# matthewhoung/inference-arena

Hardware: AMD Instinct MI355X
Metric: req/sec (whole node) + P50/P99 e2e latency, YOLOv5n→MobileNetV2 at 1/2/4/8 GPU (higher is better)
Workload: dtype fp32

## Files before the change

### csrc/bindings.cpp

```cpp
#include <pybind11/numpy.h>
#include <pybind11/pybind11.h>
#include <pybind11/stl.h>

#include <cstring>
#include <malloc.h>
#include <map>
#include <mutex>

#include "kernels/launch.h"
#include "runtime/executor.h"
#include "runtime/echo_instance.h"
#include "runtime/http_front.h"
#include "runtime/http_loadgen.h"
#include "runtime/ipc_buffer.h"
#include "runtime/peer.h"
#include "runtime/jpeg_decode.h"
#include "runtime/jpeg_ingest.h"
#include "runtime/batcher.h"
#include "runtime/split.h"
#include "runtime/crash_trace.h"

namespace py = pybind11;
using namespace arena;

// ... 28 lines not shown
  p.H = req<int>(d, "H");
  p.W = req<int>(d, "W");
  p.xs = req<int>(d, "xs");
  p.Cin = req<int>(d, "Cin");
  p.w = ptr<const void*>(d, "w");
  p.Kpad = req<int>(d, "Kpad");
  p.bias = ptr<const float*>(d, "bias");
  p.y = ptr<void*>(d, "y");
  p.Ho = req<int>(d, "Ho");
  p.Wo = req<int>(d, "Wo");
  p.ys = req<int>(d, "ys");
  p.Cout = req<int>(d, "Cout");
  p.Cout_pad = req<int>(d, "Cout_pad");
  p.KH = req<int>(d, "KH");
  p.KW = req<int>(d, "KW");
  p.stride = get<int>(d, "stride", 1);
  p.pad_t = get<int>(d, "pad_t", 0);
  p.pad_l = get<int>(d, "pad_l", 0);
  p.res = ptr<const void*>(d, "res");
  p.rs = get<int>(d, "rs", 0);
  p.y2 = ptr<void*>(d, "y2");
  p.y2s = get<int>(d, "y2s", 0);
  p.act = get<int>(d, "act", 0);
  p.f32out = get<int>(d, "f32out", 0);
  p.bdev = ptr<const int*>(d, "bdev");
  p.impl = get<int>(d, "impl", 0);
  p.pw_w = ptr<const void*>(d, "pw_w");
  p.pw_bias = ptr<const float*>(d, "pw_bias");
  p.pw_y = ptr<void*>(d, "pw_y");
  p.pw_ys = get<int>(d, "pw_ys", 0);
  p.pw_cout = get<int>(d, "pw_cout", 0);
  p.pw_kpad = get<int>(d, "pw_kpad", 0);
  p.pw_act = get<int>(d, "pw_act", 0);
  p.w3 = ptr<const void*>(d, "w3");
  p.sk_ws = ptr<float*>(d, "sk_ws");
  p.sk_ws_bytes = get<int64_t>(d, "sk_ws_bytes", 0);
  prepare_kernels();
  if (get<int>(d, "f32", 0))
    conv2d_f32(p, stream_of(d));
  else
    conv2d(p, stream_of(d));
}

void py_dwconv(const py::dict& d) {
  DwParams p{};
  p.x = ptr<const void*>(d, "x");
  p.B = req<int>(d, "B");
  p.H = req<int>(d, "H");
  p.W = req<int>(d, "W");
  p.xs = req<int>(d, "xs");
  p.C = req<int>(d, "C");
  p.w = ptr<const void*>(d, "w");
  p.bias = ptr<const float*>(d, "bias");
  p.y = ptr<void*>(d, "y");
  p.Ho = req<int>(d, "Ho");
  p.Wo = req<int>(d, "Wo");
  p.ys = req<int>(d, "ys");
  p.stride = get<int>(d, "stride", 1);
  p.act = get<int>(d, "act", 0);
  p.bdev = ptr<const int*>(d, "bdev");
  if (get<int>(d, "f32", 0))
    dwconv3x3_f32(p, stream_of(d));
  else
    dwconv3x3(p, stream_of(d));
}

// ... 444 lines not shown
  m.def("crash_trace_installed", &arena::crash_trace_installed);
  m.def("dump_thread_stack", &arena::dump_thread_stack, py::arg("tid"));
  m.def("malloc_trim", []() {
    py::gil_scoped_release nogil;
    return malloc_trim(0) != 0;
  });
  m.def("malloc_info", []() {
    const struct mallinfo2 mi = mallinfo2();
    py::dict d;
    d["arena"] = (uint64_t)mi.arena;
    d["mmapped"] = (uint64_t)mi.hblkhd;
    d["in_use"] = (uint64_t)mi.uordblks;
    d["free"] = (uint64_t)mi.fordblks;
    d["releasable"] = (uint64_t)mi.keepcost;
    return d;
  });
  bind_jpeg(m);
  m.def("conv2d", &py_conv2d);
  m.def("set_conv_impl", &set_conv_impl);
  m.def("get_conv_impl", &get_conv_impl);
  m.def("dwconv3x3", &py_dwconv);
  m.def("sppf_pool", &py_sppf);
  m.def("ir_block", &py_ir_block);
  m.def("c3_block", &py_c3_block);
  m.def("set_conv_pw", &set_conv_pw);
  m.def("set_conv_v3", &set_conv_v3);
  m.def("set_ir_wave", &set_ir_wave);
  m.def("set_irx_parts", &set_irx_parts);
  m.def("set_irx_slices_big", &set_irx_slices_big);
  m.def("set_ir_t14", &set_ir_t14);
  m.def("set_ir_crop", &set_ir_crop);
  m.def("set_ir_s2k16", &set_ir_s2k16);
  m.def("set_ir_crop_split", &set_ir_crop_split);
  m.def("letterbox_s2d", &py_letterbox);
  m.def("detect_decode", &py_decode);
  m.def("yolo_raw", &py_yolo_raw);
  m.def("tensor_in_s2d", &py_tensor_in);
  m.def("nms", &py_nms);
  m.def("crop_plan", &py_crop_plan);
  m.def("crop_gather_s2d", &py_crop_gather);
  m.def("global_avgpool", &py_avgpool);
  m.def("head_pool", &py_head_pool);
  m.def("topk_softmax", &py_topk);
  m.attr("SIZEOF_IMAGE_META") = (int)sizeof(ImageMeta);
  m.attr("SIZEOF_CTRL") = (int)sizeof(Ctrl);
  m.attr("SIZEOF_CANDIDATE") = (int)sizeof(Candidate);
  m.attr("SIZEOF_DETECTION") = (int)sizeof(Detection);
  m.attr("SIZEOF_CROPREF") = (int)sizeof(CropRef);
  m.attr("SIZEOF_TOPK") = (int)sizeof(TopkResult);
  m.attr("OP_FIELDS") = kOpFields;

  py::class_<Executor, std::shared_ptr<Executor>>(m, "Executor")
      .def(py::init([](const py::dict& cfg) { return std::make_shared<Executor>(config_from(cfg)); }))
      .def("set_weights",
           [](Executor& e, py::array_t<uint8_t, py::array::c_style> blob) { e.set_weights(blob.data(), blob.size()); })
      .def("set_weights_device",
           [](Executor& e, uintptr_t ptr, size_t bytes) {
             py::gil_scoped_release nogil;
             e.set_weights_device((const void*)ptr, bytes);
           })
      .def("weights_host",
           [](Executor& e) {
             std::vector<uint8_t> v;
             {
               py::gil_scoped_release nogil;
               v = e.weights_host();
// ... 112 lines not shown
           })
      .def("submit_device",
           [](Executor& e, const std::vector<std::tuple<uintptr_t, int, int, int>>& images,
              const std::vector<py::array_t<float, py::array::c_style | py::array::forcecast>>& boxes) {
             if (images.size() != boxes.size()) throw std::runtime_error("submit_device: one box array per image");
             std::vector<Executor::DeviceImage> imgs;
             std::vector<std::vector<Detection>> dets(images.size());
             for (size_t i = 0; i < images.size(); ++i) {
               Executor::DeviceImage d;
               d.ptr = std::get<0>(images[i]);
               d.h = std::get<1>(images[i]);
               d.w = std::get<2>(images[i]);
               d.device = std::get<3>(images[i]);
               imgs.push_back(d);
               const auto& b = boxes[i];
               if (b.size() == 0) continue;
               if (b.ndim() != 2 || b.shape(1) != 6) throw std::runtime_error("submit_device: boxes must be [k, 6]");
               const float* q = b.data();
               for (ssize_t k = 0; k < b.shape(0); ++k, q += 6) {
                 Detection dd{};
                 dd.x1 = q[0];
                 dd.y1 = q[1];
                 dd.x2 = q[2];
                 dd.y2 = q[3];
                 dd.conf = q[4];
                 dd.cls = (int)q[5];
                 dets[i].push_back(dd);
               }
             }
             py::gil_scoped_release nogil;
             return e.submit_device(imgs, dets);
           })
      .def("conv_choices", &Executor::conv_choices)
      .def("stream", &Executor::stream);

  py::class_<SplitInstance, std::shared_ptr<SplitInstance>>(m, "SplitInstance")
      .def(py::init([](std::shared_ptr<Executor> det, std::shared_ptr<Executor> cls) {
        return std::make_shared<SplitInstance>(det, cls);
      }))
      .def("submit",
           [](SplitInstance& s, const py::list& imgs) {
             std::vector<py::array> keep;
             auto v = images_from(imgs, keep);
             py::gil_scoped_release nogil;
             return s.submit(v);
           })
      .def("collect",
           [](SplitInstance& s, int slot) {
             BatchResult r;
             {
               py::gil_scoped_release nogil;
               r = s.collect(slot);
             }
             return result_to_py(r, s.max_det());
           })
      .def("num_slots", &SplitInstance::num_slots)
      .def("buckets", &SplitInstance::buckets);

  py::class_<JpegSet, std::shared_ptr<JpegSet>>(m, "JpegSet")
      .def(py::init(&make_jpeg_set), py::arg("uploads"), py::arg("pinned") = true,
           "JPEG uploads entropy-decoded once into (pinned) host buffers, for Executor.submit_jpeg_set")
      .def("__len__", [](const JpegSet& s) { return s.items.size(); })
      .def("coef_bytes", [](const JpegSet& s, int i) { return (int64_t)jpeg_payload_bytes(s.items.at(i)->info); })
      .def_property_readonly("pinned", [](const JpegSet& s) {
        for (const auto& it : s.items)
          if (!it->pinned) return false;
// ... 443 lines not shown
```

### csrc/kernels/halo_x3g.hip

```cpp
#include <stdexcept>
#include <string>

#include "common.h"
#include "launch.h"

namespace arena {

namespace {

typedef float f32x16 __attribute__((ext_vector_type(16)));
typedef unsigned u32x4 __attribute__((ext_vector_type(4)));

constexpr int HG_P = 56;

__host__ __device__ constexpr int hg_th(int TW, int WM, int TM) { return WM * TM * (32 / TW); }
__host__ __device__ constexpr int hg_lds_bytes(int TW, int WM, int WN, int TM, int TN) {
  return ((hg_th(TW, WM, TM) + 2) * (TW + 2) + 2 * WN * TN * 32) * HG_P * 2;
}
__host__ __device__ constexpr int hr_lds_bytes(int TW, int WM, int TM) {
  return (hg_th(TW, WM, TM) + 2) * (TW + 2) * HG_P * 2;
}

__device__ __forceinline__ int hg_xcd_remap(int bx, int nx) {
  const int q = nx / 8, r = nx % 8, x = bx % 8, y = bx / 8;
  return (x < r ? x * (q + 1) : r * (q + 1) + (x - r) * q) + y;
}

__device__ __forceinline__ f32x16 hg_mfma_x3(const bf16x8& ah, const bf16x8& am, const bf16x8& al,
                                             const bf16x8& bh, const bf16x8& bm, const bf16x8& bl, f32x16 c) {
  c = __builtin_amdgcn_mfma_f32_32x32x16_bf16(am, bm, c, 0, 0, 0);
  c = __builtin_amdgcn_mfma_f32_32x32x16_bf16(al, bh, c, 0, 0, 0);
  c = __builtin_amdgcn_mfma_f32_32x32x16_bf16(ah, bl, c, 0, 0, 0);
  c = __builtin_amdgcn_mfma_f32_32x32x16_bf16(am, bh, c, 0, 0, 0);
  c = __builtin_amdgcn_mfma_f32_32x32x16_bf16(ah, bm, c, 0, 0, 0);
  return __builtin_amdgcn_mfma_f32_32x32x16_bf16(ah, bh, c, 0, 0, 0);
}

}

template <int TW, int WM, int WN, int TM, int TN, int PWN>
__device__ __forceinline__ void hg_epilogue(const ConvParams& p, f32x16 (&acc)[TM][TN], int b, int oy0, int ox0,
                                            int n0, int wm, int wn, int lane) {
  constexpr int RF = 32 / TW, BN = WN * TN * 32;
  const int fr = lane & 31, fk = 8 * (lane >> 5);
  const int kh4 = 4 * (lane >> 5);
  if constexpr (PWN > 0) {
// ... 96 lines not shown
  }
}

template <int TW, int WM, int WN, int TM, int TN, int PWN = 0>
__global__ __launch_bounds__(WM * WN * 64) void conv_x3hg_kernel(const ConvParams p) {
  static_assert(PWN == 0 || WN == 1, "the fused 1x1 needs every 3x3 channel of a pixel in one wave");
  constexpr int NT = WM * WN * 64;
  constexpr int RF = 32 / TW;
  constexpr int TH = WM * TM * RF;
  constexpr int HC = TW + 2, HPIX = (TH + 2) * HC;
  constexpr int BN = WN * TN * 32;
  constexpr int XI = (HPIX * 4 + NT - 1) / NT;
  constexpr int WI = (BN * 6 + NT - 1) / NT;
  extern __shared__ __attribute__((aligned(16))) bf16 hg_lds[];
  bf16* sX = hg_lds;
  bf16* sW = hg_lds + HPIX * HG_P;

  const int tid = threadIdx.x, lane = tid & 63, wave = tid >> 6;
  const int wm = wave % WM, wn = wave / WM;
  const int tiles_x = (p.Wo + TW - 1) / TW, tiles_y = (p.Ho + TH - 1) / TH;
  const int ntn = (p.Cout_pad + BN - 1) / BN;
  const int per_img = tiles_x * tiles_y * ntn;
  const int bx = hg_xcd_remap(blockIdx.x, gridDim.x);
  const int b = bx / per_img;
  if (b >= live_batch(p.B, p.bdev)) return;
  int t = bx - b * per_img;
  const int nt = t % ntn;
  t /= ntn;
  const int ty = t / tiles_x, tx = t - ty * tiles_x;
  const int oy0 = ty * TH, ox0 = tx * TW, n0 = nt * BN;
  const int iy0 = oy0 - p.pad_t, ix0 = ox0 - p.pad_l;
  const int H = p.H, W = p.W, Cin = p.Cin;

  const __amdgpu_buffer_rsrc_t xr = __builtin_amdgcn_make_buffer_rsrc(
      const_cast<void*>(p.x), (short)0, (int)((size_t)p.B * H * W * p.xs * 4), 0x00020000);
  const int cin32 = (Cin + 31) >> 5;
  const __amdgpu_buffer_rsrc_t wr = __builtin_amdgcn_make_buffer_rsrc(
      const_cast<void*>(p.w3), (short)0, (int)((size_t)9 * cin32 * p.Cout_pad * 192), 0x00020000);
  constexpr int kOob = 0x7fffffff & ~15;

  int x_off[XI];
  const size_t img = (size_t)b * H * W;
#pragma unroll
  for (int j = 0; j < XI; ++j) {
    const int i = tid + NT * j;
    const int px = i >> 2, q = i & 3;
    const int hy = px / HC, hx = px - hy * HC;
    const int iy = iy0 + hy, ix = ix0 + hx;
    const bool in = i < HPIX * 4 && (unsigned)iy < (unsigned)H && (unsigned)ix < (unsigned)W;
    x_off[j] = in ? (int)(((img + (size_t)iy * W + ix) * p.xs + 4 * q) * 4) : kOob;
  }
  int w_off[WI];
#pragma unroll
  for (int j = 0; j < WI; ++j) {
    const int i = tid + NT * j;
    const int row = i / 6, piece = i - (i / 6) * 6;
    const int n = n0 + row;
    w_off[j] = (i < BN * 6 && n < p.Cout_pad) ? (n * 96 + (piece >> 1) * 32 + 8 * (piece & 1)) * 2 : kOob;
  }

  f32x4 rx[XI];
  u32x4 rw[WI];
  auto load_x = [&](int cc) {
#pragma unroll
    for (int j = 0; j < XI; ++j) {
      const int i = tid + NT * j;
// ... 311 lines not shown
  X(1, 16, 4, 1, 1, 2)   \
  X(2, 16, 4, 1, 2, 3)   \
  X(3, 16, 4, 1, 1, 3)   \
  X(4, 16, 4, 1, 1, 5)   \
  X(5, 16, 8, 1, 1, 5)   \
  X(6, 8, 4, 1, 1, 2)    \
  X(7, 8, 4, 1, 1, 5)    \
  X(8, 16, 2, 2, 2, 1)   \
  X(9, 8, 4, 1, 1, 3)

#define HR_PW_VARIANTS(X) \
  X(0, 16, 4, 1, 2, 2)  \
  X(1, 16, 4, 2, 2, 2)  \
  X(2, 16, 4, 1, 3, 3)  \
  X(3, 16, 4, 2, 3, 3)  \
  X(4, 8, 4, 1, 2, 2)   \
  X(5, 8, 4, 1, 3, 3)

}

bool x3hg_supported(const ConvParams& p) {
  const size_t x_bytes = (size_t)p.B * p.H * p.W * p.xs * 4;
  const size_t w_bytes = (size_t)9 * ((p.Cin + 31) / 32) * p.Cout_pad * 192;
  return p.w3 != nullptr && p.KH == 3 && p.KW == 3 && p.stride == 1 && p.Cin % 4 == 0 && p.xs % 4 == 0 &&
         x_bytes < (1u << 31) - (1u << 20) && w_bytes < (1u << 31) - (1u << 20) && p.Cout % 4 == 0 &&
         p.ys % 4 == 0 && (p.res == nullptr || p.rs % 4 == 0) && (p.y2 == nullptr || p.y2s % 4 == 0) &&
         p.lb_meta == nullptr && p.pw_w == nullptr;
}

bool x3hg_pw_supported(const ConvParams& p, int bn, int pwn) {
  return p.w3 != nullptr && p.KH == 3 && p.KW == 3 && p.stride == 1 && p.Cin % 4 == 0 && p.xs % 4 == 0 &&
         (size_t)p.B * p.H * p.W * p.xs * 4 < (1u << 31) - (1u << 20) && p.Cout % 4 == 0 && p.Cout_pad <= bn &&
         p.res == nullptr && p.y2 == nullptr && p.lb_meta == nullptr && p.pw_w != nullptr && p.pw_y != nullptr &&
         p.pw_kpad == bn && p.pw_cout % 4 == 0 && p.pw_cout <= 32 * pwn && p.pw_ys % 4 == 0;
}

bool conv_x3hg_pw(const ConvParams& p, hipStream_t s, int v) {
  switch (v) {
#define HG_PW_CASE(V, TW, WM, TM, TN, PWN) \
  case V:                                 \
    if (!x3hg_pw_supported(p, TN * 32, PWN)) return false; \
    hg_launch<TW, WM, 1, TM, TN, PWN>(p, s);                \
    return true;
    HG_PW_VARIANTS(HG_PW_CASE)
#undef HG_PW_CASE
    default: return false;
  }
}

bool conv_x3hg(const ConvParams& p, hipStream_t s, int v) {
  if (!x3hg_supported(p)) return false;
  switch (v) {
#define HG_CASE(V, TW, WM, WN, TM, TN) \
  case V: hg_launch<TW, WM, WN, TM, TN>(p, s); return true;
    HG_VARIANTS(HG_CASE)
#undef HG_CASE
    default: return false;
  }
}

bool conv_x3hr(const ConvParams& p, hipStream_t s, int v) {
  if (!x3hg_supported(p)) return false;
  switch (v) {
#define HR_CASE(V, TW, WM, WN, TM, TN) \
  case V: hr_launch<TW, WM, WN, TM, TN>(p, s); return true;
    HR_VARIANTS(HR_CASE)
#undef HR_CASE
// ... 44 lines not shown
```

### csrc/kernels/launch.h

```cpp
#pragma once
#include <hip/hip_runtime.h>
#include <stdint.h>
#include <stdexcept>
#include <string>

namespace arena {

struct ImageMeta;
struct CropRef;
struct Ctrl;
struct ConvParams {
  const void* x;
  int B, H, W;
  int xs;
  int Cin;
  const void* w;
  int Kpad;
  const float* bias;
  void* y;
  int Ho, Wo, ys;
  int Cout;
  int Cout_pad;
  int KH, KW, stride, pad_t, pad_l;
  const void* res;
  int rs;
  void* y2;
  int y2s;
  int act;
  int f32out;
  const int* bdev;
  int impl;
  const void* pw_w;
  const float* pw_bias;
  void* pw_y;
  int pw_ys, pw_cout, pw_kpad, pw_act;
  const uint8_t* lb_pool;
  const ImageMeta* lb_meta;
  const void* w3;
  float* sk_ws;
  int64_t sk_ws_bytes;
  int sk_splits;
};
void conv2d(const ConvParams& p, hipStream_t s);
void conv_igemm(const ConvParams& p, hipStream_t s);
bool conv_pw(const ConvParams& p, hipStream_t s);
void set_conv_pw(bool v);
bool conv3x3_v3(const ConvParams& p, hipStream_t s);
bool conv_fc(const ConvParams& p, hipStream_t s);
void set_conv_v3(bool v);
void set_conv_impl(int v);
int get_conv_impl();

constexpr int kF32Variants = 16;
constexpr int kF32X3 = 40;
constexpr int kF32X3Variants = 12;
constexpr int kF32Halo = 100;
constexpr int kF32X3Halo = 101;
constexpr int kF32X3HaloN3 = 102;
constexpr int kF32X3HaloN2 = 103;
constexpr int kF32Stream = 104;
constexpr int kF32StreamN2 = 105;
constexpr int kF32Fc = 106;
constexpr int kF32StreamExact = 107;
constexpr int kF32X3Halo16 = 108;
constexpr int kF32X3Halo16N3 = 109;
constexpr int kF32X3H16 = 110;
constexpr int kF32X3G = 111;
constexpr int kF32X3GVariants = 20;
// ... 336 lines not shown
```

### csrc/runtime/executor.cpp

```cpp
#include "executor.h"
#include "peer.h"

#include <pthread.h>
#include <sys/prctl.h>

#include <algorithm>
#include <chrono>
#include <cmath>
#include <cstdio>
#include <cstdlib>
#include <cstring>
#include <thread>
#include <stdexcept>
#include <string>

#include "../kernels/common.h"
#include "../kernels/jpeg_desc.h"
#include "jpeg_decode.h"
#include "trace.h"

namespace arena {

namespace {
float bits_to_float(int64_t v) {
  uint32_t u = (uint32_t)v;
  float f;
  std::memcpy(&f, &u, 4);
  return f;
}
size_t align_up(size_t v, size_t a) { return (v + a - 1) / a * a; }
constexpr size_t kCtrlBytes = 256;
}

Executor::Executor(const ExecutorConfig& cfg) : cfg_(cfg) {
  if (cfg_.max_batch <= 0 || cfg_.max_batch > 1024) throw std::runtime_error("Executor: max_batch out of range");
  if (cfg_.cand_cap > 16384) throw std::runtime_error("Executor: cand_cap > 16384");
  ARENA_HIP_CHECK(hipSetDevice(cfg_.device));
  prepare_kernels();
  max_B_ = cfg_.max_batch;
  {
    int khz = 0;
    if (hipDeviceGetAttribute(&khz, hipDeviceAttributeWallClockRate, cfg_.device) == hipSuccess && khz > 0)
      wall_khz_ = (double)khz;
  }
  {
    const char* e = std::getenv("ARENA_DEBUG_SYNC");
    debug_sync_ = e != nullptr ? std::atoi(e) : 0;
    const char* at = std::getenv("ARENA_AUTOTUNE");
    autotune_ = at != nullptr ? std::atoi(at) : 1;
    const char* c = std::getenv("ARENA_COPY_MODE");
    copy_mode_ = c != nullptr && std::atoi(c) == 2 ? 2 : 0;
    const char* cc = std::getenv("ARENA_CONCURRENT");
    concurrent_ = cc != nullptr ? std::atoi(cc) : 1;
    if (debug_sync_) concurrent_ = 0;
    const char* ns = std::getenv("ARENA_SLOTS");
    n_slots_ = concurrent_ ? std::min(kMaxSlots, std::max(2, ns != nullptr ? std::atoi(ns) : 4)) : 2;
    const char* nc = std::getenv("ARENA_CONCURRENCY");
    n_streams_ = concurrent_ ? std::min(n_slots_, std::max(1, nc != nullptr ? std::atoi(nc) : 3)) : 1;
    const char* sg = std::getenv("ARENA_STAGGER");
    if (concurrent_ && n_streams_ > 1) {
      std::string spec = sg != nullptr ? sg : "0.25";
      for (size_t a = 0; a < spec.size();) {
        size_t e = spec.find(',', a);
        if (e == std::string::npos) e = spec.size();
        const double f = std::atof(spec.substr(a, e - a).c_str());
// ... 169 lines not shown
}

void Executor::set_weights_device(const void* dev, size_t bytes) {
  ARENA_HIP_CHECK(hipSetDevice(cfg_.device));
  if (d_weights_ == nullptr || bytes != weights_bytes_)
    throw std::runtime_error("set_weights_device: only a same-size update of uploaded weights is supported");
  sync_slots();
  ARENA_HIP_CHECK(hipMemcpy(d_weights_, dev, bytes, hipMemcpyDeviceToDevice));
}

std::vector<uint8_t> Executor::weights_host() {
  std::vector<uint8_t> out(weights_bytes_);
  if (d_weights_ == nullptr || weights_bytes_ == 0) return out;
  ARENA_HIP_CHECK(hipSetDevice(cfg_.device));
  sync_slots();
  ARENA_HIP_CHECK(hipMemcpy(out.data(), d_weights_, weights_bytes_, hipMemcpyDeviceToHost));
  return out;
}

void Executor::set_program(const int64_t* ops, int n_ops, const int64_t* cls_ops, int n_cls_ops) {
  prog_.resize(n_ops);
  for (int i = 0; i < n_ops; ++i) std::memcpy(prog_[i].data(), ops + (size_t)i * kOpFields, sizeof(OpRecord));
  cls_prog_.resize(n_cls_ops);
  for (int i = 0; i < n_cls_ops; ++i)
    std::memcpy(cls_prog_[i].data(), cls_ops + (size_t)i * kOpFields, sizeof(OpRecord));
  has_topk_ = has_det_ = has_raw_ = has_stamps_ = false;
  for (const auto& r : prog_) {
    has_topk_ |= r[0] == OP_TOPK;
    has_stamps_ |= r[0] == OP_STAMP;
    has_det_ |= r[0] == OP_NMS || r[0] == OP_CROPPLAN;
    for (int f = 1; f < kOpFields; ++f) has_raw_ |= r[f] == BUF_RAWOUT && (r[0] == OP_YOLORAW || r[0] == OP_CONV);
  }
  if (has_raw_ && cfg_.raw_out_bytes <= 0) throw std::runtime_error("program exports raw outputs: raw_out_bytes = 0");
}

int Executor::crop_cap_for(int B) const { return std::max(cfg_.min_crop_cap, B * cfg_.crop_cap_per_image); }

std::vector<int> Executor::buckets() const {
  std::vector<int> r;
  for (auto& kv : buckets_) r.push_back(kv.first);
  return r;
}

uintptr_t Executor::arena_ptr(int B) const {
  auto it = buckets_.find(B);
  return it == buckets_.end() ? 0 : (uintptr_t)it->second.d_arena[0];
}

void Executor::read_arena(int B, int64_t offset, void* dst, size_t bytes) {
  auto it = buckets_.find(B);
  if (it == buckets_.end()) throw std::runtime_error("read_arena: unknown bucket");
  if (offset < 0 || offset + (int64_t)bytes > it->second.info.arena_bytes)
    throw std::runtime_error("read_arena: range outside the arena");
  ARENA_HIP_CHECK(hipSetDevice(cfg_.device));
  sync_slots();
  ARENA_HIP_CHECK(hipMemcpy(dst, it->second.d_arena[it->second.last_slot] + offset, bytes, hipMemcpyDeviceToHost));
}

void Executor::add_bucket(int B, const int64_t* offsets, int n_buffers, int64_t arena_bytes,
                          const std::vector<int>* impl) {
  if (B <= 0 || B > max_B_) throw std::runtime_error("add_bucket: B outside (0, max_batch]");
  if (prog_.empty()) throw std::runtime_error("add_bucket: set_program first");
  if (d_weights_ == nullptr) throw std::runtime_error("add_bucket: set_weights first");
  ARENA_HIP_CHECK(hipSetDevice(cfg_.device));
  Bucket& bk = buckets_[B];
  bk.info.B = B;
// ... 128 lines not shown
}

bool Executor::lanes_for(const Bucket& bk) const {
  if (bk.info.B > lanes_max_batch()) return false;
  for (const OpRecord& r : prog_)
    if (r[kLaneField] >= 1 && r[kLaneField] <= kMaxLanes) return true;
  return false;
}

int64_t Executor::sk_lane_bytes() {
  static const int64_t v = [] {
    const char* e = std::getenv("ARENA_SPLITK_WS_MB");
    return (int64_t)std::max(1, e != nullptr ? std::atoi(e) : 16) << 20;
  }();
  return v;
}

void Executor::destroy_graphs(Bucket& bk, int s) {
  if (bk.graph[s]) hipGraphExecDestroy(bk.graph[s]);
  bk.graph[s] = nullptr;
  for (hipGraphExec_t g : bk.parts[s])
    if (g) hipGraphExecDestroy(g);
  bk.parts[s].clear();
  for (auto& sg : bk.segs[s])
    if (sg.g) hipGraphExecDestroy(sg.g);
  bk.segs[s].clear();
}

void Executor::capture(Bucket& bk, int s) {
  Slot& sl = slots_[s];
  hipStream_t st = sl.stream;
  ARENA_HIP_CHECK(hipStreamSynchronize(st));
  destroy_graphs(bk, s);
  auto capture_range = [&](size_t a, size_t b) {
    std::vector<OpRecord> part(prog_.begin() + a, prog_.begin() + b);
    hipGraph_t g = nullptr;
    hipGraphExec_t ge = nullptr;
    ARENA_HIP_CHECK(hipStreamBeginCapture(st, hipStreamCaptureModeThreadLocal));
    try {
      enqueue_program(part, bk, sl, st, (int)a);
    } catch (...) {
      hipStreamEndCapture(st, &g);
      if (g) hipGraphDestroy(g);
      throw;
    }
    ARENA_HIP_CHECK(hipStreamEndCapture(st, &g));
    ARENA_HIP_CHECK(hipGraphInstantiate(&ge, g, nullptr, nullptr, 0));
    ARENA_HIP_CHECK(hipGraphDestroy(g));
    return ge;
  };
  if (!lanes_for(bk)) {
    std::vector<size_t> cuts{0};
    if (bk.info.B >= 16)
      for (double f : stagger_) {
        const size_t k = (size_t)std::lround(f * (double)prog_.size());
        if (k > cuts.back() && k < prog_.size()) cuts.push_back(k);
      }
    if (cuts.size() > 1) {
      cuts.push_back(prog_.size());
      for (size_t i = 0; i + 1 < cuts.size(); ++i) bk.parts[s].push_back(capture_range(cuts[i], cuts[i + 1]));
    } else {
      bk.graph[s] = capture_range(0, prog_.size());
    }
    return;
  }
  ensure_lanes(sl);
  auto lane_of = [&](size_t i) {
    const int64_t l = prog_[i][kLaneField];
// ... 51 lines not shown
    if (!forked[l]) {
      if (!fork_recorded) {
        ARENA_HIP_CHECK(hipEventRecord(sl.fork_ev, st));
        fork_recorded = true;
      }
      ARENA_HIP_CHECK(hipStreamWaitEvent(sl.lane_stream[l], sl.fork_ev, 0));
      forked[l] = true;
    }
    ARENA_HIP_CHECK(hipGraphLaunch(sg.g, sl.lane_stream[l]));
  }
  join();
}

uint8_t* Executor::resolve(Bucket& bk, Slot& sl, int64_t buf, int64_t coff, int eb) {
  uint8_t* base = nullptr;
  switch (buf) {
    case BUF_NONE: return nullptr;
    case BUF_CTRL: base = sl.d_in; break;
    case BUF_META: base = sl.d_in + kCtrlBytes; break;
    case BUF_POOL: base = sl.d_in + in_bytes_meta(); break;
    case BUF_DETCOUNT: base = sl.d_out; break;
    case BUF_DET: base = sl.d_out + out_off_det(); break;
    case BUF_TOPK: base = sl.d_out + out_off_topk(); break;
    case BUF_RAWOUT: base = sl.d_out + out_off_raw(); break;
    case BUF_XCROPS: base = sl.d_out + out_off_xcrops(); break;
    default:
      if (buf < 0 || buf >= (int64_t)bk.info.offsets.size())
        throw std::runtime_error("program references unknown buffer " + std::to_string(buf));
      base = bk.d_arena[sl.idx] + bk.info.offsets[buf];
  }
  return base + coff * eb;
}

void Executor::enqueue_program(const std::vector<OpRecord>& prog, Bucket& bk, Slot& sl, hipStream_t s_main,
                               int op_offset, int force_impl) {
  Ctrl* ctrl = (Ctrl*)resolve(bk, sl, BUF_CTRL, 0, 1);
  const ImageMeta* meta = (const ImageMeta*)resolve(bk, sl, BUF_META, 0, 1);
  const uint8_t* pool = resolve(bk, sl, BUF_POOL, 0, 1);
  const int B = bk.info.B, CC = bk.info.crop_cap;
  auto batch = [&](int64_t kind) { return kind == BATCH_CROPS ? CC : B; };
  auto bdev = [&](int64_t kind) -> const int* { return kind == BATCH_CROPS ? &ctrl->n_crops : &ctrl->n_images; };
  const uint8_t* W = d_weights_;

  for (size_t oi = 0; oi < prog.size(); ++oi) {
    const OpRecord& r = prog[oi];
    hipStream_t s = s_main;
    const bool f32 = r[kDtypeField] == 1;
    const int eb = f32 ? 4 : 2;
    switch (r[0]) {
      case OP_CONV: {
        ConvParams p{};
        const size_t gi = (size_t)op_offset + oi;
        p.impl = force_impl ? force_impl : (gi < bk.impl.size() ? bk.impl[gi] : 0);
        p.x = resolve(bk, sl, r[1], r[2], eb);
        p.xs = (int)r[3];
        p.H = (int)r[4];
        p.W = (int)r[5];
        p.Cin = (int)r[6];
        p.w = W + r[7];
        p.Kpad = (int)r[8];
        p.bias = (const float*)(W + r[9]);
        p.f32out = (int)r[29];
        p.y = resolve(bk, sl, r[10], r[11], p.f32out ? 4 : eb);
        p.ys = (int)r[12];
        p.Ho = (int)r[13];
        p.Wo = (int)r[14];
        p.Cout = (int)r[15];
        p.Cout_pad = (int)r[16];
        p.KH = (int)r[17];
        p.KW = (int)r[18];
        p.stride = (int)r[19];
        p.pad_t = (int)r[20];
        p.pad_l = (int)r[21];
        p.res = resolve(bk, sl, r[22], r[23], eb);
        p.rs = (int)r[24];
        p.y2 = resolve(bk, sl, r[25], r[26], eb);
        p.y2s = (int)r[27];
        p.act = (int)r[28];
        p.B = batch(r[30]);
        p.bdev = bdev(r[30]);
        if (r[41] != 0) p.w3 = W + r[40];
        {
          const int64_t ln = r[kLaneField];
          const int li = ln >= 1 && ln <= kMaxLanes ? (int)ln : 0;
          p.sk_ws = (float*)((uint8_t*)sl.sk_ws + (size_t)li * sk_lane_bytes());
          p.sk_ws_bytes = sk_lane_bytes();
        }
        if (r[1] == BUF_POOL) {
          if (!f32 || r[30] != 0) throw std::runtime_error("executor: letterbox-source conv must be fp32 over images");
          p.x = nullptr;
          p.lb_pool = pool;
          p.lb_meta = meta;
          p.impl = kF32X3H16;
        }
        if (r[34] > 0) {
          p.pw_w = W + r[31];
          p.pw_kpad = (int)r[32];
          p.pw_bias = (const float*)(W + r[33]);
          p.pw_cout = (int)r[34];
          p.pw_y = resolve(bk, sl, r[36], r[37], eb);
          p.pw_ys = (int)r[38];
          p.pw_act = (int)r[39];
          if (!f32) p.impl = 2;
        }
        if (f32)
          conv2d_f32(p, s);
        else
          conv2d(p, s);
        break;
      }
      case OP_DWCONV: {
        DwParams p{};
        p.x = resolve(bk, sl, r[1], r[2], eb);
        p.xs = (int)r[3];
        p.H = (int)r[4];
        p.W = (int)r[5];
        p.C = (int)r[6];
        p.w = W + r[7];
        p.bias = (const float*)(W + r[8]);
        p.y = resolve(bk, sl, r[9], r[10], eb);
        p.ys = (int)r[11];
        p.Ho = (int)r[12];
        p.Wo = (int)r[13];
        p.stride = (int)r[14];
        p.act = (int)r[15];
        p.B = batch(r[16]);
        p.bdev = bdev(r[16]);
        if (f32)
          dwconv3x3_f32(p, s);
        else
          dwconv3x3(p, s);
        break;
      }
      case OP_IRBLOCK: {
        IrParams p{};
        p.x = resolve(bk, sl, r[1], r[2], eb);
// ... 868 lines not shown
```

### csrc/runtime/executor.h

```cpp
#pragma once
#include <chrono>
#include <hip/hip_runtime.h>

#include <array>
#include <atomic>
#include <condition_variable>
#include <cstdint>
#include <functional>
#include <map>
#include <mutex>
#include <thread>
#include <vector>

#include "../kernels/launch.h"
#include "instance.h"

namespace arena {

constexpr int kOpFields = 48;
constexpr int kDtypeField = 47;
constexpr int kLaneField = 46;
constexpr int kMaxLanes = 3;
constexpr int kMaxSlots = 6;
constexpr int kMaxStaggerParts = 5;
constexpr int kMaxEstBuckets = 257;
using OpRecord = std::array<int64_t, kOpFields>;

enum OpType : int64_t {
  OP_CONV = 1,
  OP_DWCONV = 2,
  OP_SPPF = 3,
  OP_LETTERBOX = 4,
  OP_ZERO = 5,
  OP_DECODE = 6,
  OP_NMS = 7,
  OP_CROPPLAN = 8,
  OP_CROPGATHER = 9,
  OP_AVGPOOL = 10,
  OP_TOPK = 11,
  OP_TENSORIN = 12,
  OP_YOLORAW = 13,
  OP_IRBLOCK = 14,
  OP_STEMFUSED = 15,
  OP_C3FUSED = 16,
  OP_HEADPOOL = 17,
  OP_STAMP = 18,
};

enum ReservedBuf : int64_t {
  BUF_NONE = -1,
  BUF_CTRL = -10,
  BUF_META = -11,
  BUF_POOL = -12,
  BUF_DET = -13,
  BUF_DETCOUNT = -14,
  BUF_TOPK = -15,
  BUF_RAWOUT = -16,
  BUF_XCROPS = -17,
};
// ... 79 lines not shown
  struct Slot {
    uint8_t* d_in = nullptr;
    uint8_t* d_out = nullptr;
    float* sk_ws = nullptr;
    uint8_t* h_in = nullptr;
    size_t h_cap = 0;
    uint8_t* h_out = nullptr;
    hipEvent_t copied = nullptr, started = nullptr, done = nullptr;
    hipEvent_t phase[kMaxStaggerParts] = {};
    hipStream_t stream = nullptr;
    hipStream_t lane_stream[kMaxLanes] = {};
    hipEvent_t fork_ev = nullptr, lane_ev[kMaxLanes] = {};
    int idx = 0;
    std::chrono::steady_clock::time_point t_submit{};
    bool polled = false;
    std::chrono::steady_clock::time_point t_poll{};
    bool busy = false;
    int bucket = 0;
    int n_images = 0;
    size_t in_used = 0;
  };
  struct Bucket {
    BucketInfo info;
    uint8_t* d_arena[kMaxSlots] = {};
    int last_slot = 0;
    hipGraphExec_t graph[kMaxSlots] = {};
    std::vector<hipGraphExec_t> parts[kMaxSlots];
    struct Seg {
      int lane = 0;
      hipGraphExec_t g = nullptr;
    };
    std::vector<Seg> segs[kMaxSlots];
    std::vector<int16_t> impl;
  };

  void alloc_slots();
  void ensure_lanes(Slot& sl);
  void sync_slots();
  void free_arenas(Bucket& bk);
  void capture(Bucket& bk, int slot);
  void wait_done(Slot& sl);
  void note_done(Slot& sl);
  void release_copy(Slot& sl);
  static int64_t sk_lane_bytes();
  uint64_t copy_release_n_ = 0;
  void launch_graph(Bucket& bk, int slot, hipStream_t st, int n_live = -1);
  void destroy_graphs(Bucket& bk, int slot);
  bool lanes_for(const Bucket& bk) const;
  void enqueue_program(const std::vector<OpRecord>& prog, Bucket& bk, Slot& sl, hipStream_t s,
                       int op_offset = 0, int force_impl = 0);
  void autotune(Bucket& bk);

 public:
  std::vector<int> conv_choices(int B) const {
    auto it = buckets_.find(B);
    if (it == buckets_.end()) return {};
    return std::vector<int>(it->second.impl.begin(), it->second.impl.end());
  }

 private:
  void enqueue_results_d2h(Bucket& bk, Slot& sl, int n);
  uint8_t* resolve(Bucket& bk, Slot& sl, int64_t buf, int64_t coff_elems, int elem_bytes);
  int pick_bucket(int n) const;
  size_t in_bytes_meta() const;
  size_t jpeg_desc_off() const;
  size_t pool_cap() const;
  size_t in_bytes_total() const;
  size_t out_off_det() const;
  size_t out_off_topk() const;
  size_t out_bytes_total() const;
  size_t out_off_raw() const;
  size_t out_off_xcrops() const;
  size_t out_off_stamps() const;
  int acquire_slot();
  void parallel_copy(std::vector<std::function<void()>>& jobs);

  ExecutorConfig cfg_;
  int max_B_ = 0;
  hipStream_t compute_ = nullptr, copy_ = nullptr;
  uint8_t* d_weights_ = nullptr;
  size_t weights_bytes_ = 0;
  std::vector<OpRecord> prog_, cls_prog_;
  std::map<int, Bucket> buckets_;
  Slot slots_[kMaxSlots];
  int n_slots_ = 2;
  int next_slot_ = 0;
  hipStream_t streams_[kMaxSlots] = {};
  int n_streams_ = 1;
  uint64_t seq_ = 0;
  std::vector<double> stagger_;
  int stagger_min_batch_ = 32;
  int last_launched_ = -1;
  bool has_topk_ = false, has_det_ = false, has_raw_ = false, has_stamps_ = false;
  double wall_khz_ = 100000.0;
  bool peer_stage_ = false;
  std::vector<int> peer_enabled_;
  void enable_peer(int src, const char* what);
  int copy_mode_ = 0;
  int concurrent_ = 1;
  int autotune_ = 1;
  int debug_sync_ = 0;
  std::mutex mu_;
  std::vector<std::thread> workers_;
  std::mutex pool_mu_;
  std::condition_variable pool_cv_, pool_done_cv_;
  std::vector<std::function<void()>>* pool_jobs_ = nullptr;
  std::atomic<int> pool_next_{0};
  std::atomic<float> wall_est_us_[kMaxEstBuckets] = {};
  int pool_active_ = 0;
  uint64_t pool_gen_ = 0;
  bool pool_stop_ = false;
};

}
```

### inference_arena_amd/ops/functional.py

```python
from __future__ import annotations

import ctypes
import struct

import numpy as np
import torch

from ..engine.planner import ACT, pack_conv_weight, pack_conv_weight_x3
from . import native

IMAGE_META = struct.Struct("<qiiiiiif12x")


def _stream() -> int:
    return torch.cuda.current_stream().cuda_stream


def _ptr(t: torch.Tensor | None, elem_off: int = 0) -> int:
    if t is None:
        return 0
    return t.data_ptr() + elem_off * t.element_size()


def pack_weights(w: torch.Tensor, b: torch.Tensor, device, dtype: str = "bf16"):
    wb, bb, kpad, cpad = pack_conv_weight(w.detach().cpu().float(), b.detach().cpu().float(), dtype)
    wt = torch.frombuffer(bytearray(wb), dtype=torch.float32 if dtype == "fp32" else torch.bfloat16).to(device)
    bt = torch.frombuffer(bytearray(bb), dtype=torch.float32).to(device)
    w3 = None
    if dtype == "fp32":
        w3 = torch.frombuffer(bytearray(pack_conv_weight_x3(w.detach().cpu().float())), dtype=torch.int16).to(device)
    return wt, bt, kpad, cpad, w3


def conv2d_nhwc(x: torch.Tensor, w: torch.Tensor, b: torch.Tensor, *, stride: int = 1, pad=None, act=None,
                x_coff: int = 0, cin: int | None = None, out: torch.Tensor | None = None, out_coff: int = 0,
                res: torch.Tensor | None = None, res_coff: int = 0, out2: torch.Tensor | None = None,
                out2_coff: int = 0, f32out: bool = False, out_hw=None, bdev: torch.Tensor | None = None,
                packed=None, impl: int = 0, pw=None) -> torch.Tensor:
    f32 = x.dtype == torch.float32
    B, H, W, Cx = x.shape
    cout, cin_w, kh, kw = w.shape
    cin = cin or cin_w
    if pad is None:
        pad = (kh // 2, kw // 2)
    if isinstance(pad, int):
        pad = (pad, pad)
    if out_hw is None:
        Ho = (H + 2 * pad[0] - kh) // stride + 1
        Wo = (W + 2 * pad[1] - kw) // stride + 1
    else:
        Ho, Wo = out_hw
    if out is None:
        out = torch.empty(B, Ho, Wo, cout, dtype=torch.float32 if (f32out or f32) else torch.bfloat16, device=x.device)
    wt, bt, kpad, cpad, w3 = packed if packed is not None else pack_weights(w, b, x.device, "fp32" if f32 else "bf16")
    pwd = {}
    if pw is not None:
        from ..engine.planner import pack_pw_weight_x3

        if not f32:
            raise ValueError("conv2d_nhwc: the functional fused pointwise path is fp32-only")
        w2, b2 = pw
        co2 = w2.shape[0]
        k2 = (cout + 31) // 32 * 32
        w2p = torch.frombuffer(bytearray(pack_pw_weight_x3(w2.detach().cpu().float(), k2)),
                               dtype=torch.int16).to(x.device)
        b2p = torch.zeros((co2 + 15) // 16 * 16)
        b2p[:co2] = b2.detach().float()
        b2p = b2p.to(x.device)
        out = torch.empty(B, Ho, Wo, co2, dtype=torch.float32, device=x.device)
        pwd = {"pw_w": _ptr(w2p), "pw_bias": _ptr(b2p), "pw_y": _ptr(out), "pw_ys": co2, "pw_cout": co2,
               "pw_kpad": k2, "pw_act": 0}
    skd = {}
    if 171 <= int(impl) < 180:
        ws = torch.empty(8 * B * Ho * Wo * cpad, dtype=torch.float32, device=x.device)
        skd = {"sk_ws": _ptr(ws), "sk_ws_bytes": ws.numel() * 4}
    native().conv2d({
        "x": _ptr(x, x_coff), "B": B, "H": H, "W": W, "xs": Cx, "Cin": cin,
        "w": _ptr(wt), "Kpad": kpad, "bias": _ptr(bt),
        "y": _ptr(out, out_coff), "Ho": Ho, "Wo": Wo, "ys": out.shape[-1], "Cout": cout, "Cout_pad": cpad,
        "KH": kh, "KW": kw, "stride": stride, "pad_t": pad[0], "pad_l": pad[1],
        "res": _ptr(res, res_coff), "rs": res.shape[-1] if res is not None else 0,
        "y2": _ptr(out2, out2_coff), "y2s": out2.shape[-1] if out2 is not None else 0,
        "act": ACT[act], "f32out": int(f32out), "bdev": _ptr(bdev), "stream": _stream(), "f32": int(f32),
        "impl": int(impl), "w3": _ptr(w3), **pwd, **skd,
    })
    if pw is not None:
        torch.cuda.synchronize(x.device)
    return out


def dwconv3x3_nhwc(x: torch.Tensor, w: torch.Tensor, b: torch.Tensor, *, stride: int = 1, act="relu6",
                   bdev: torch.Tensor | None = None) -> torch.Tensor:
    B, H, W, C = x.shape
    f32 = x.dtype == torch.float32
    Ho, Wo = (H - 1) // stride + 1, (W - 1) // stride + 1
    y = torch.empty(B, Ho, Wo, C, dtype=x.dtype, device=x.device)
    wt = w.detach().float().reshape(C, 9).t().contiguous().to(x.dtype).to(x.device)
    bt = b.detach().float().contiguous().to(x.device)
    native().dwconv3x3({"x": _ptr(x), "B": B, "H": H, "W": W, "xs": C, "C": C, "w": _ptr(wt), "bias": _ptr(bt),
                        "y": _ptr(y), "Ho": Ho, "Wo": Wo, "ys": C, "stride": stride, "act": ACT[act],
                        "bdev": _ptr(bdev), "stream": _stream(), "f32": int(f32)})
    return y


# ... 135 lines not shown
```

### inference_arena_amd/utils/settings.py

```python
from __future__ import annotations

import functools
import os
from pathlib import Path

from pydantic import BaseModel


def _read_dotenv(path: Path) -> dict[str, str]:
    out: dict[str, str] = {}
    if not path.exists():
        return out
    for line in path.read_text(encoding="utf-8").splitlines():
        line = line.strip()
        if not line or line.startswith("#") or "=" not in line:
            continue
        k, v = line.split("=", 1)
        v = v.strip()
        if v[:1] in ("'", '"') and v[0] in v[1:]:
            v = v[1:v.index(v[0], 1)]
        else:
            v = v.split(" #", 1)[0].split("\t#", 1)[0].strip()
        out[k.strip()] = v
    return out


class Settings(BaseModel):
    LOG_LEVEL: str = "INFO"
    PORT: int = 8100
    HOST: str = "0.0.0.0"
    MODELS_DIR: str = "model_repository"
    LABELS_FILE: str = ""
    CLASSIFICATION_GRPC_ENDPOINT: str = "127.0.0.1:8201"
    TRITON_GRPC_ENDPOINT: str = "127.0.0.1:8001"
    TRITON_HTTP_ENDPOINT: str = "127.0.0.1:8000"
    TRITON_TIMEOUT_SECONDS: float = 60.0
    ARENA_DEVICE: str = "gpu"
    ARENA_GPU: int = 0
    ARENA_GPUS: str = ""
    ARENA_CLS_GPU: int = -1
    ARENA_MAX_BATCH: int = 32
    ARENA_QUEUE_DELAY_US: int = 500
    ARENA_DECODE_THREADS: int = 8
    ARENA_CONFIDENCE: str = ""
    ARENA_CROP_TRANSPORT: str = "jpeg"
    ARENA_DEVICE_RING_SLOTS: int = 512
    ARENA_CROP_ENCODE: str = "pil"
    ARENA_FANOUT: str = "parallel"
    ARENA_GATEWAY_MODE: str = "pipeline"
    ARENA_INSTANCES: int = 1
    ARENA_WEIGHT_SEED: int = 0
    ARENA_FAULT_EVERY: int = 0
    ARENA_INFER_SERVICE: int = 0
    ARENA_IR_S2K16: int = 1

    @classmethod
    def from_env(cls, env_file: str | Path = ".env", **overrides) -> "Settings":
        vals: dict[str, str] = _read_dotenv(Path(env_file))
        for k in cls.model_fields:
            if k in os.environ:
                vals[k] = os.environ[k]
        vals.update({k: v for k, v in overrides.items() if v is not None})
        return cls(**vals)


@functools.lru_cache
def get_settings() -> Settings:
    return Settings.from_env()
```

Before: 10710.

## Gate detection-head box conv tiles on class logits below the confidence threshold

Detection-head conv pairs that feed the decode op are found by matching op records. For each pair, the class conv is reordered to run before the box conv. The fused x3hg 3x3+1x1 box kernel then reads the class logits for its output tile and exits the whole block early when no logit reaches a threshold derived from the decode confidence cutoff (logit minus a small margin). This avoids box-regression compute for spatial tiles that decode would discard anyway. The cost is an extra global gate read per block and unwritten box outputs for skipped tiles, which is correct only as long as decode ignores those positions.

Measured after the change: 11060 (median of 6 runs). +3.2%, better.

```diff
diff --git a/csrc/bindings.cpp b/csrc/bindings.cpp
--- a/csrc/bindings.cpp
+++ b/csrc/bindings.cpp
@@ -84,6 +84,9 @@
   p.pw_cout = get<int>(d, "pw_cout", 0);
   p.pw_kpad = get<int>(d, "pw_kpad", 0);
   p.pw_act = get<int>(d, "pw_act", 0);
+  p.gate = ptr<const float*>(d, "gate");
+  p.gate_n = get<int>(d, "gate_n", 0);
+  p.gate_min = get<float>(d, "gate_min", 0.f);
   p.w3 = ptr<const void*>(d, "w3");
   p.sk_ws = ptr<float*>(d, "sk_ws");
   p.sk_ws_bytes = get<int64_t>(d, "sk_ws_bytes", 0);
@@ -594,6 +597,28 @@
   m.def("set_ir_crop", &set_ir_crop);
   m.def("set_ir_s2k16", &set_ir_s2k16);
   m.def("set_ir_crop_split", &set_ir_crop_split);
+  m.def("set_head_gate", &set_head_gate);
+  m.def("get_head_gate", &get_head_gate);
+  m.def(
+      "head_gate_min",
+      [](float conf_thr) -> py::object {
+        float g;
+        if (!head_gate_min(conf_thr, &g)) return py::none();
+        return py::float_(g);
+      },
+      py::arg("conf_thr"), "the gate's logit threshold for a confidence threshold (float32); None: the gate is off");
+  m.def(
+      "head_gate_pairs",
+      [](py::array_t<int64_t, py::array::c_style> ops) {
+        if (ops.ndim() != 2 || ops.shape(1) != kOpFields) throw std::runtime_error("ops must be int64 [n, OP_FIELDS]");
+        py::list out;
+        for (const HeadGatePair& gp : head_gate_pairs(ops.data(), (int)ops.shape(0), kOpFields))
+          out.append(py::make_tuple(gp.box, gp.cls, gp.level));
+        return out;
+      },
+      py::arg("ops"), "[(box conv op, class conv op, level)] of a program's records");
+  m.attr("HEAD_BOX_CHANNELS") = kHeadBoxChannels;
+  m.attr("HEAD_CLS_CHANNELS") = kHeadClsChannels;
   m.def("letterbox_s2d", &py_letterbox);
   m.def("detect_decode", &py_decode);
   m.def("yolo_raw", &py_yolo_raw);
@@ -772,6 +797,9 @@
              return e.submit_device(imgs, dets);
            })
       .def("conv_choices", &Executor::conv_choices)
+      .def("exec_order", &Executor::exec_order, py::arg("B"),
+           "program op indices in the order bucket B's graphs launch them")
+      .def("gated_ops", &Executor::gated_ops, py::arg("B"), "ops of bucket B that run with a tile gate")
       .def("stream", &Executor::stream);
 
   py::class_<SplitInstance, std::shared_ptr<SplitInstance>>(m, "SplitInstance")
diff --git a/csrc/kernels/halo_x3g.hip b/csrc/kernels/halo_x3g.hip
--- a/csrc/kernels/halo_x3g.hip
+++ b/csrc/kernels/halo_x3g.hip
@@ -12,6 +12,7 @@
 typedef unsigned u32x4 __attribute__((ext_vector_type(4)));
 
 constexpr int HG_P = 56;
+constexpr int HG_GATE_MAX_N = 80;
 
 __host__ __device__ constexpr int hg_th(int TW, int WM, int TM) { return WM * TM * (32 / TW); }
 __host__ __device__ constexpr int hg_lds_bytes(int TW, int WM, int WN, int TM, int TN) {
@@ -174,6 +175,30 @@
   const int iy0 = oy0 - p.pad_t, ix0 = ox0 - p.pad_l;
   const int H = p.H, W = p.W, Cin = p.Cin;
 
+  if constexpr (PWN > 0) {
+    if (p.gate != nullptr) {
+      constexpr int GJ = (TH * TW * (HG_GATE_MAX_N / 4) + NT - 1) / NT;
+      const int nq = p.gate_n >> 2;
+      const int items = TH * TW * nq;
+      const float gm = p.gate_min;
+      const float nan = __builtin_nanf("");
+      float4 gv[GJ];
+#pragma unroll
+      for (int j = 0; j < GJ; ++j) {
+        const int i = tid + NT * j;
+        const int px = i / nq, q = i - px * nq;
+        const int oy = oy0 + px / TW, ox = ox0 + px % TW;
+        gv[j] = make_float4(nan, nan, nan, nan);
+        if (i < items && oy < p.Ho && ox < p.Wo)
+          gv[j] = *(const float4*)(p.gate + (((size_t)b * p.Ho + oy) * p.Wo + ox) * p.pw_ys + 4 * q);
+      }
+      int any = 0;
+#pragma unroll
+      for (int j = 0; j < GJ; ++j) any |= gv[j].x >= gm || gv[j].y >= gm || gv[j].z >= gm || gv[j].w >= gm;
+      if (!__syncthreads_or(any)) return;
+    }
+  }
+
   const __amdgpu_buffer_rsrc_t xr = __builtin_amdgcn_make_buffer_rsrc(
       const_cast<void*>(p.x), (short)0, (int)((size_t)p.B * H * W * p.xs * 4), 0x00020000);
   const int cin32 = (Cin + 31) >> 5;
@@ -551,7 +576,10 @@
   return p.w3 != nullptr && p.KH == 3 && p.KW == 3 && p.stride == 1 && p.Cin % 4 == 0 && p.xs % 4 == 0 &&
          (size_t)p.B * p.H * p.W * p.xs * 4 < (1u << 31) - (1u << 20) && p.Cout % 4 == 0 && p.Cout_pad <= bn &&
          p.res == nullptr && p.y2 == nullptr && p.lb_meta == nullptr && p.pw_w != nullptr && p.pw_y != nullptr &&
-         p.pw_kpad == bn && p.pw_cout % 4 == 0 && p.pw_cout <= 32 * pwn && p.pw_ys % 4 == 0;
+         p.pw_kpad == bn && p.pw_cout % 4 == 0 && p.pw_cout <= 32 * pwn && p.pw_ys % 4 == 0 &&
+         (p.gate == nullptr ||
+          (p.gate_n > 0 && p.gate_n <= HG_GATE_MAX_N && p.gate_n % 4 == 0 && p.gate_n <= p.pw_ys &&
+           (uintptr_t)p.gate % 16 == 0));
 }
 
 bool conv_x3hg_pw(const ConvParams& p, hipStream_t s, int v) {
diff --git a/csrc/kernels/launch.h b/csrc/kernels/launch.h
--- a/csrc/kernels/launch.h
+++ b/csrc/kernels/launch.h
@@ -34,6 +34,9 @@
   const float* pw_bias;
   void* pw_y;
   int pw_ys, pw_cout, pw_kpad, pw_act;
+  const float* gate;
+  int gate_n;
+  float gate_min;
   const uint8_t* lb_pool;
   const ImageMeta* lb_meta;
   const void* w3;
diff --git a/csrc/runtime/executor.cpp b/csrc/runtime/executor.cpp
--- a/csrc/runtime/executor.cpp
+++ b/csrc/runtime/executor.cpp
@@ -30,7 +30,17 @@
 }
 size_t align_up(size_t v, size_t a) { return (v + a - 1) / a * a; }
 constexpr size_t kCtrlBytes = 256;
-}
+static_assert(kHgOpConv == OP_CONV && kHgOpDecode == OP_DECODE && kHgDtypeField == kDtypeField &&
+                  sizeof(OpRecord) == sizeof(int64_t) * kOpFields,
+              "head_gate.h reads the executor's op records");
+bool g_head_gate = [] {
+  const char* e = std::getenv("ARENA_HEAD_GATE");
+  return e == nullptr || std::atoi(e) != 0;
+}();
+}
+
+void set_head_gate(bool v) { g_head_gate = v; }
+bool get_head_gate() { return g_head_gate; }
 
 Executor::Executor(const ExecutorConfig& cfg) : cfg_(cfg) {
   if (cfg_.max_batch <= 0 || cfg_.max_batch > 1024) throw std::runtime_error("Executor: max_batch out of range");
@@ -266,6 +276,7 @@
     for (int f = 1; f < kOpFields; ++f) has_raw_ |= r[f] == BUF_RAWOUT && (r[0] == OP_YOLORAW || r[0] == OP_CONV);
   }
   if (has_raw_ && cfg_.raw_out_bytes <= 0) throw std::runtime_error("program exports raw outputs: raw_out_bytes = 0");
+  gate_pairs_ = head_gate_pairs(prog_.empty() ? nullptr : prog_[0].data(), n_ops, kOpFields);
 }
 
 int Executor::crop_cap_for(int B) const { return std::max(cfg_.min_crop_cap, B * cfg_.crop_cap_per_image); }
@@ -460,8 +471,20 @@
   hipStream_t st = sl.stream;
   ARENA_HIP_CHECK(hipStreamSynchronize(st));
   destroy_graphs(bk, s);
+  if (s == 0) {
+    bk.exec_order.clear();
+    bk.gated.clear();
+  }
   auto capture_range = [&](size_t a, size_t b) {
     std::vector<OpRecord> part(prog_.begin() + a, prog_.begin() + b);
+    if (s == 0) {
+      std::vector<const HeadGatePair*> gate;
+      const std::vector<size_t> order = exec_plan(part, bk, (int)a, 0, gate);
+      for (size_t k = 0; k < order.size(); ++k) {
+        bk.exec_order.push_back((int)(a + order[k]));
+        if (gate[k] != nullptr) bk.gated.push_back((int)(a + order[k]));
+      }
+    }
     hipGraph_t g = nullptr;
     hipGraphExec_t ge = nullptr;
     ARENA_HIP_CHECK(hipStreamBeginCapture(st, hipStreamCaptureModeThreadLocal));
@@ -579,6 +602,29 @@
   return base + coff * eb;
 }
 
+std::vector<size_t> Executor::exec_plan(const std::vector<OpRecord>& prog, const Bucket& bk, int op_offset,
+                                        int force_impl, std::vector<const HeadGatePair*>& gate) const {
+  std::vector<size_t> order(prog.size());
+  for (size_t k = 0; k < order.size(); ++k) order[k] = k;
+  gate.assign(prog.size(), nullptr);
+  if (!g_head_gate || force_impl != 0) return order;
+  for (const HeadGatePair& gp : gate_pairs_) {
+    const long li = (long)gp.box - op_offset;
+    float gm;
+    if (li < 0 || li + 1 >= (long)prog.size() || gp.cls >= (int)prog_.size()) continue;
+    if (!head_gate_min(gp.conf_thr, &gm)) continue;
+    if (prog[li] != prog_[gp.box] || prog[li + 1] != prog_[gp.cls]) continue;
+    const int impl = gp.box < (int)bk.impl.size() ? bk.impl[gp.box] : 0;
+    const bool x3hg_pw = impl == 0 || (impl >= kF32X3HGPw && impl < kF32X3HGPw + kF32X3HGPwVariants) ||
+                         (impl >= kF32X3HGPwSmall && impl < kF32X3HGPwSmall + kF32X3HGPwSmallVariants);
+    if (!x3hg_pw) continue;
+    order[li] = (size_t)li + 1;
+    order[li + 1] = (size_t)li;
+    gate[li + 1] = &gp;
+  }
+  return order;
+}
+
 void Executor::enqueue_program(const std::vector<OpRecord>& prog, Bucket& bk, Slot& sl, hipStream_t s_main,
                                int op_offset, int force_impl) {
   Ctrl* ctrl = (Ctrl*)resolve(bk, sl, BUF_CTRL, 0, 1);
@@ -589,7 +635,10 @@
   auto bdev = [&](int64_t kind) -> const int* { return kind == BATCH_CROPS ? &ctrl->n_crops : &ctrl->n_images; };
   const uint8_t* W = d_weights_;
 
-  for (size_t oi = 0; oi < prog.size(); ++oi) {
+  std::vector<const HeadGatePair*> gate;
+  const std::vector<size_t> order = exec_plan(prog, bk, op_offset, force_impl, gate);
+  for (size_t k = 0; k < prog.size(); ++k) {
+    const size_t oi = order[k];
     const OpRecord& r = prog[oi];
     hipStream_t s = s_main;
     const bool f32 = r[kDtypeField] == 1;
@@ -649,6 +698,11 @@
           p.pw_ys = (int)r[38];
           p.pw_act = (int)r[39];
           if (!f32) p.impl = 2;
+          if (gate[k] != nullptr) {
+            p.gate = (const float*)resolve(bk, sl, r[36], r[37] + kHeadBoxChannels, eb);
+            p.gate_n = kHeadClsChannels;
+            head_gate_min(gate[k]->conf_thr, &p.gate_min);
+          }
         }
         if (f32)
           conv2d_f32(p, s);
diff --git a/csrc/runtime/executor.h b/csrc/runtime/executor.h
--- a/csrc/runtime/executor.h
+++ b/csrc/runtime/executor.h
@@ -13,6 +13,7 @@
 #include <vector>
 
 #include "../kernels/launch.h"
+#include "head_gate.h"
 #include "instance.h"
 
 namespace arena {
@@ -25,6 +26,9 @@
 constexpr int kMaxStaggerParts = 5;
 constexpr int kMaxEstBuckets = 257;
 using OpRecord = std::array<int64_t, kOpFields>;
+
+void set_head_gate(bool v);
+bool get_head_gate();
 
 enum OpType : int64_t {
   OP_CONV = 1,
@@ -170,6 +174,7 @@
     };
     std::vector<Seg> segs[kMaxSlots];
     std::vector<int16_t> impl;
+    std::vector<int> exec_order, gated;
   };
 
   void alloc_slots();
@@ -188,8 +193,18 @@
   void enqueue_program(const std::vector<OpRecord>& prog, Bucket& bk, Slot& sl, hipStream_t s,
                        int op_offset = 0, int force_impl = 0);
   void autotune(Bucket& bk);
+  std::vector<size_t> exec_plan(const std::vector<OpRecord>& prog, const Bucket& bk, int op_offset, int force_impl,
+                                std::vector<const HeadGatePair*>& gate) const;
 
  public:
+  std::vector<int> exec_order(int B) const {
+    auto it = buckets_.find(B);
+    return it == buckets_.end() ? std::vector<int>{} : it->second.exec_order;
+  }
+  std::vector<int> gated_ops(int B) const {
+    auto it = buckets_.find(B);
+    return it == buckets_.end() ? std::vector<int>{} : it->second.gated;
+  }
   std::vector<int> conv_choices(int B) const {
     auto it = buckets_.find(B);
     if (it == buckets_.end()) return {};
@@ -219,6 +234,7 @@
   uint8_t* d_weights_ = nullptr;
   size_t weights_bytes_ = 0;
   std::vector<OpRecord> prog_, cls_prog_;
+  std::vector<HeadGatePair> gate_pairs_;
   std::map<int, Bucket> buckets_;
   Slot slots_[kMaxSlots];
   int n_slots_ = 2;
diff --git a/csrc/runtime/head_gate.h b/csrc/runtime/head_gate.h
--- /dev/null
+++ b/csrc/runtime/head_gate.h
@@ -0,0 +1,71 @@
+#pragma once
+#include <cmath>
+#include <cstdint>
+#include <cstring>
+#include <vector>
+
+namespace arena {
+
+constexpr int kHeadBoxChannels = 64;
+constexpr int kHeadClsChannels = 80;
+
+constexpr double kHeadGateMargin = 1.0 / 64.0;
+constexpr float kHeadGateThrMin = 1e-3f;
+constexpr float kHeadGateThrMax = 0.999f;
+
+inline bool head_gate_min(float conf_thr, float* gate_min) {
+  if (!(conf_thr >= kHeadGateThrMin && conf_thr <= kHeadGateThrMax)) return false;
+  const double t = (double)conf_thr;
+  const double g = std::log(t / (1.0 - t)) - kHeadGateMargin;
+  float f = (float)g;
+  if ((double)f > g) f = std::nextafterf(f, -INFINITY);
+  *gate_min = f;
+  return true;
+}
+
+constexpr int64_t kHgOpConv = 1, kHgOpDecode = 6;
+constexpr int kHgDtypeField = 47;
+
+struct HeadGatePair {
+  int box;
+  int cls;
+  int level;
+  float conf_thr;
+};
+
+inline std::vector<HeadGatePair> head_gate_pairs(const int64_t* ops, int n, int fields) {
+  std::vector<HeadGatePair> out;
+  if (ops == nullptr || fields <= kHgDtypeField) return out;
+  auto rec = [&](int i) { return ops + (size_t)i * fields; };
+  for (int d = 0; d < n; ++d) {
+    const int64_t* dr = rec(d);
+    if (dr[0] != kHgOpDecode || dr[kHgDtypeField] != 1) continue;
+    uint32_t bits = (uint32_t)dr[18];
+    float thr;
+    std::memcpy(&thr, &bits, 4);
+    for (int l = 0; l < 3; ++l) {
+      const int64_t buf = dr[1 + 4 * l], coff = dr[2 + 4 * l], cs = dr[3 + 4 * l], hw = dr[4 + 4 * l];
+      if (buf < 0) continue;
+      for (int i = 0; i + 1 < d; ++i) {
+        const int64_t* a = rec(i);
+        const int64_t* c = rec(i + 1);
+        if (a[0] != kHgOpConv || a[kHgDtypeField] != 1 || c[0] != kHgOpConv || c[kHgDtypeField] != 1) continue;
+        if (!(a[34] == kHeadBoxChannels && a[36] == buf && a[37] == coff && a[38] == cs && a[13] == hw && a[14] == hw))
+          continue;
+        const bool c_pw = c[34] > 0;
+        const int64_t cb = c_pw ? c[36] : c[10], cc = c_pw ? c[37] : c[11], cst = c_pw ? c[38] : c[12];
+        const int64_t cn = c_pw ? c[34] : c[15];
+        if (!(cn == kHeadClsChannels && cb == buf && cc == coff + kHeadBoxChannels && cst == cs && c[13] == hw &&
+              c[14] == hw && c[30] == a[30]))
+          continue;
+        const bool disjoint = a[1] != c[1] || a[2] + a[6] <= c[2] || c[2] + c[6] <= a[2];
+        if (!disjoint || a[1] == buf || c[1] == buf || a[22] >= 0 || c[22] >= 0) continue;
+        out.push_back(HeadGatePair{i, i + 1, l, thr});
+        break;
+      }
+    }
+  }
+  return out;
+}
+
+}
diff --git a/inference_arena_amd/ops/functional.py b/inference_arena_amd/ops/functional.py
--- a/inference_arena_amd/ops/functional.py
+++ b/inference_arena_amd/ops/functional.py
@@ -36,7 +36,8 @@
                 x_coff: int = 0, cin: int | None = None, out: torch.Tensor | None = None, out_coff: int = 0,
                 res: torch.Tensor | None = None, res_coff: int = 0, out2: torch.Tensor | None = None,
                 out2_coff: int = 0, f32out: bool = False, out_hw=None, bdev: torch.Tensor | None = None,
-                packed=None, impl: int = 0, pw=None) -> torch.Tensor:
+                packed=None, impl: int = 0, pw=None, pw_out: torch.Tensor | None = None, pw_out_coff: int = 0,
+                gate=None) -> torch.Tensor:
     f32 = x.dtype == torch.float32
     B, H, W, Cx = x.shape
     cout, cin_w, kh, kw = w.shape
@@ -67,9 +68,24 @@
         b2p = torch.zeros((co2 + 15) // 16 * 16)
         b2p[:co2] = b2.detach().float()
         b2p = b2p.to(x.device)
-        out = torch.empty(B, Ho, Wo, co2, dtype=torch.float32, device=x.device)
-        pwd = {"pw_w": _ptr(w2p), "pw_bias": _ptr(b2p), "pw_y": _ptr(out), "pw_ys": co2, "pw_cout": co2,
-               "pw_kpad": k2, "pw_act": 0}
+        if pw_out is None:
+            out = torch.empty(B, Ho, Wo, co2, dtype=torch.float32, device=x.device)
+            pw_out_coff = 0
+        else:
+            out = pw_out
+            if (out.shape[:3] != (B, Ho, Wo) or out.shape[3] < pw_out_coff + co2 or out.dtype != torch.float32
+                    or out.device != x.device or not out.is_contiguous()):
+                raise ValueError(f"conv2d_nhwc: pw_out {tuple(out.shape)} {out.dtype} does not fit the 1x1 output")
+        pwd = {"pw_w": _ptr(w2p), "pw_bias": _ptr(b2p), "pw_y": _ptr(out, pw_out_coff), "pw_ys": out.shape[-1],
+               "pw_cout": co2, "pw_kpad": k2, "pw_act": 0}
+        if gate is not None:
+            gt, gcoff, gn, gmin = gate
+            if (gt.shape != out.shape or gt.dtype != torch.float32 or gt.device != x.device or not gt.is_contiguous()
+                    or gcoff < 0 or gn <= 0 or gcoff + gn > gt.shape[3]):
+                raise ValueError("conv2d_nhwc: the gate logits must match the 1x1 output tensor's shape and stride")
+            pwd.update({"gate": _ptr(gt, gcoff), "gate_n": int(gn), "gate_min": float(gmin)})
+    elif gate is not None or pw_out is not None:
+        raise ValueError("conv2d_nhwc: gate / pw_out need pw")
     skd = {}
     if 171 <= int(impl) < 180:
         ws = torch.empty(8 * B * Ho * Wo * cpad, dtype=torch.float32, device=x.device)
diff --git a/inference_arena_amd/utils/settings.py b/inference_arena_amd/utils/settings.py
--- a/inference_arena_amd/utils/settings.py
+++ b/inference_arena_amd/utils/settings.py
@@ -53,6 +53,7 @@
     ARENA_FAULT_EVERY: int = 0
     ARENA_INFER_SERVICE: int = 0
     ARENA_IR_S2K16: int = 1
+    ARENA_HEAD_GATE: int = 1
 
     @classmethod
     def from_env(cls, env_file: str | Path = ".env", **overrides) -> "Settings":
```
